# yanivw12/gs2mesh

Hardware: AMD Instinct MI355X
Metric: stereo-pair renders/sec + TSDF Mvoxel-updates/sec (higher is better)
Workload: dtype f32

## Files before the change

### gs2mesh_amd/_lib.py

```python
from __future__ import annotations

import ctypes as C

import numpy as np
import os

_HERE = os.path.dirname(os.path.abspath(__file__))
LIB_PATH = os.path.join(_HERE, "libgs2mesh_amd.so")

vp = C.c_void_p
i32 = C.c_int
i64 = C.c_int64
f32 = C.c_float
f64 = C.c_double


class Camera(C.Structure):
    _fields_ = [("width", C.c_int32), ("height", C.c_int32), ("tanfovx", f32), ("tanfovy", f32),
                ("viewmatrix", f32 * 16), ("projmatrix", f32 * 16), ("campos", f32 * 3)]


class Gaussians(C.Structure):
    _fields_ = [("P", C.c_int32), ("sh_degree", C.c_int32), ("M", C.c_int32), ("raw", C.c_int32),
                ("xyz", vp), ("scales", vp), ("rotations", vp), ("opacities", vp), ("shs", vp), ("shs_rest", vp)]
# ... 41 lines not shown
    "gs2m_raster_status": (i32, [vp, vp, i32, C.POINTER(i64), C.POINTER(i32), C.POINTER(i64)]),
    "gs2m_raster_stage_times": (i32, [vp, vp, C.POINTER(f64), C.POINTER(i64)]),
    "gs2m_raster_blend_cycles": (i32, [vp, vp, C.POINTER(C.c_uint64)]),
    "gs2m_raster_download_geometry": (i32, [vp, vp, i32, i32, vp, vp, vp, vp, vp, vp]),
    "gs2m_raster_download_binning": (i32, [vp, vp, i32, i64, vp, C.c_int32, vp]),
    "gs2m_tsdf_extract_count": (i32, [vp, vp, C.POINTER(i64)]),
    "gs2m_tsdf_extract": (i32, [vp, vp, i64, vp, vp, C.POINTER(i64)]),
    "gs2m_tsdf_extract_indexed": (i32, [vp, vp, i64, vp, vp, vp, C.POINTER(i64)]),
    "gs2m_stereo_depth_occlusion": (i32, [vp, vp, i32, i32, f64, f64, vp, vp, vp]),
    "gs2m_stereo_sgm_scratch_bytes": (i64, [i32, i32, i32]),
    "gs2m_stereo_sgm": (i32, [vp, vp, i32, i32, i32, i32, i32, vp, vp, vp, i64, vp, vp]),
    "gs2m_knn_scratch_bytes": (i64, [i32]),
    "gs2m_knn_mean_dist2": (i32, [i32, vp, vp, vp, i64, vp, vp]),
    "gs2m_mask_preprocess": (i32, [i32, i32, i32, C.POINTER(vp), C.POINTER(vp), i32, i32, i32, i32, C.POINTER(vp), vp, vp]),
    "gs2m_tsdf_create": (i32, [C.POINTER(vp), f64, f64, i32, i32, i32, i64, i32]),
    "gs2m_tsdf_destroy": (i32, [vp]),
    "gs2m_tsdf_reset": (i32, [vp, vp]),
    "gs2m_tsdf_integrate": (i32, [vp, vp, vp, vp, i32, i32, f64, f64, f64, f64, C.POINTER(f64), f64, f64, f64, vp]),
    "gs2m_tsdf_integrate_batch": (i32, [vp, i32, C.POINTER(vp), C.POINTER(vp), C.POINTER(vp), i32, i32, f64, f64, f64, f64,
                                        C.POINTER(f64), f64, f64, f64, vp]),
    "gs2m_tsdf_set_stage_timing": (i32, [vp, i32]),
    "gs2m_tsdf_stage_times": (i32, [vp, vp, C.POINTER(f64), C.POINTER(i64)]),
    "gs2m_tsdf_status": (i32, [vp, vp, C.POINTER(i64), C.POINTER(i64), C.POINTER(i32)]),
    "gs2m_tsdf_download": (i32, [vp, vp, i64, vp, vp, vp, vp]),
    "gs2m_tsdf_block_keys": (i32, [vp, i64, vp, vp]),
    "gs2m_tsdf_flags_device": (i32, [vp, vp, vp]),
    "gs2m_tsdf_pack_sum": (i32, [vp, vp, i64, vp, vp]),
    "gs2m_tsdf_unpack_sum": (i32, [vp, vp, i64, vp, i32, vp]),
    "gs2m_tsdf_pack": (i32, [vp, vp, i64, i32, vp, vp, vp]),
    "gs2m_tsdf_extract_mesh": (i32, [vp, vp, C.POINTER(i64), C.POINTER(i64)]),
    "gs2m_tsdf_mesh_copy": (i32, [vp, vp, vp, vp, vp, vp]),
    "gs2m_mesh_cluster": (i32, [i32, vp, i64, vp, vp, vp, C.POINTER(i64)]),
    "gs2m_mesh_vertex_normals": (i32, [i32, vp, i64, vp, i64, vp, vp, vp]),
    "gs2m_tsdf_replace": (i32, [vp, vp, i64, i32, vp, vp, vp]),
    "gs2m_tsdf_map_bytes": (i64, [C.POINTER(C.c_int32), i32]),
    "gs2m_tsdf_block_map": (i32, [vp, C.POINTER(C.c_int32), C.POINTER(C.c_int32), i32, i32, i64, i64, i32, vp, vp]),
    "gs2m_tsdf_map_keys": (i32, [vp, C.POINTER(C.c_int32), C.POINTER(C.c_int32), i32, vp, vp, i64, C.POINTER(C.c_uint8), vp]),
    "gs2m_tsdf_unpack": (i32, [vp, vp, i64, i32, vp, vp, i32, vp]),
    "gs2m_png_create": (i32, [C.POINTER(vp), i32]),
    "gs2m_png_destroy": (i32, [vp]),
    "gs2m_png_max_bytes": (i64, [i32, i32, i32]),
    "gs2m_png_encode": (i32, [vp, i32, i32, i32, vp, i64, vp, i64, vp, i32, i32, vp]),
}

SYMBOLS = tuple(_PROTOS)

# ... 94 lines not shown
```

### gs2mesh_amd/csrc/tsdf_api.hip

```cpp
#include <math.h>
#include <stdio.h>
#include <string.h>

#include <mutex>
#include <vector>

#include "../../include/gs2mesh_amd.h"
#include "tsdf_common.h"
#include "tsdf_internal.h"
#include "roctx_ranges.h"

#define HIPCHK(expr)                                                                          \
    do {                                                                                      \
        hipError_t e__ = (expr);                                                              \
        if (e__ != hipSuccess) {                                                              \
            gs2m_set_error("%s failed: %s (%s:%d)", #expr, hipGetErrorString(e__), __FILE__, __LINE__); \
            return 1;                                                                         \
        }                                                                                     \
    } while (0)

struct gs2m_tsdf {
    int device = 0;
    double voxel_length = 0, sdf_trunc = 0, unit_length = 0;
    int color_type = 1, resolution = 16, stride = 4;
// ... 6 lines not shown
    unsigned* d_blk_tris = nullptr;
    unsigned long long* d_ntri = nullptr;
    double* mesh_v = nullptr;
    double* mesh_c = nullptr;
    int* mesh_e = nullptr;
    int* mesh_tri = nullptr;
    int64_t mesh_nv = 0, mesh_nt = 0;
    size_t mesh_cap_v = 0, mesh_cap_t = 0;
    char* mesh_scratch = nullptr;
    size_t mesh_scratch_cap = 0;
    int timing = 0;
    struct EvPair {
        int stage;
        hipEvent_t a, b;
        int frames;
    };
    std::vector<EvPair> ev_live;
    std::vector<hipEvent_t> ev_free;
    TsdfBatchFrame* d_bframes = nullptr;
    static const int kRing = 8;
    TsdfBatchFrame* h_bframes = nullptr;
    hipEvent_t ring_done[8] = {nullptr, nullptr, nullptr, nullptr, nullptr, nullptr, nullptr, nullptr};
    unsigned ring_next = 0;
};

static hipEvent_t tsdf_ev_get(gs2m_tsdf* t) {
    if (!t->ev_free.empty()) {
        hipEvent_t e = t->ev_free.back();
        t->ev_free.pop_back();
        return e;
    }
    hipEvent_t e;
    if (hipEventCreate(&e) != hipSuccess) return nullptr;
    return e;
}

static bool invert4x4(const double* m, double* inv) {
    double a[16];
    a[0] = m[5] * m[10] * m[15] - m[5] * m[11] * m[14] - m[9] * m[6] * m[15] + m[9] * m[7] * m[14] + m[13] * m[6] * m[11] - m[13] * m[7] * m[10];
    a[4] = -m[4] * m[10] * m[15] + m[4] * m[11] * m[14] + m[8] * m[6] * m[15] - m[8] * m[7] * m[14] - m[12] * m[6] * m[11] + m[12] * m[7] * m[10];
    a[8] = m[4] * m[9] * m[15] - m[4] * m[11] * m[13] - m[8] * m[5] * m[15] + m[8] * m[7] * m[13] + m[12] * m[5] * m[11] - m[12] * m[7] * m[9];
    a[12] = -m[4] * m[9] * m[14] + m[4] * m[10] * m[13] + m[8] * m[5] * m[14] - m[8] * m[6] * m[13] - m[12] * m[5] * m[10] + m[12] * m[6] * m[9];
    a[1] = -m[1] * m[10] * m[15] + m[1] * m[11] * m[14] + m[9] * m[2] * m[15] - m[9] * m[3] * m[14] - m[13] * m[2] * m[11] + m[13] * m[3] * m[10];
    a[5] = m[0] * m[10] * m[15] - m[0] * m[11] * m[14] - m[8] * m[2] * m[15] + m[8] * m[3] * m[14] + m[12] * m[2] * m[11] - m[12] * m[3] * m[10];
    a[9] = -m[0] * m[9] * m[15] + m[0] * m[11] * m[13] + m[8] * m[1] * m[15] - m[8] * m[3] * m[13] - m[12] * m[1] * m[11] + m[12] * m[3] * m[9];
    a[13] = m[0] * m[9] * m[14] - m[0] * m[10] * m[13] - m[8] * m[1] * m[14] + m[8] * m[2] * m[13] + m[12] * m[1] * m[10] - m[12] * m[2] * m[9];
// ... 8 lines not shown
    double det = m[0] * a[0] + m[1] * a[4] + m[2] * a[8] + m[3] * a[12];
    if (det == 0) return false;
    det = 1.0 / det;
    for (int i = 0; i < 16; i++) inv[i] = a[i] * det;
    return true;
}

static int zero_state(gs2m_tsdf* t, hipStream_t st, bool whole_pool, long long keep_first = -1) {
    TsdfVolume& V = t->V;
    if (whole_pool) {
        HIPCHK(hipMemsetAsync(V.tsdf, 0, sizeof(float) * (size_t)V.max_blocks * GS2M_TSDF_VOX, st));
        HIPCHK(hipMemsetAsync(V.weight, 0, sizeof(float) * (size_t)V.max_blocks * GS2M_TSDF_VOX, st));
        if (V.rgb) HIPCHK(hipMemsetAsync(V.rgb, 0, sizeof(unsigned) * 3 * (size_t)V.max_blocks * GS2M_TSDF_VOX, st));
        HIPCHK(hipMemsetAsync(V.halo, 0, (size_t)V.max_blocks, st));
    } else if (keep_first < 0) {
        gs2m_launch_tsdf_clear_used(st, V);
    } else {
        gs2m_launch_tsdf_clear_from(st, V, (unsigned)keep_first);
    }
    HIPCHK(hipMemsetAsync(V.hash_keys, 0xff, sizeof(unsigned long long) * (size_t)V.hash_cap, st));
    HIPCHK(hipMemsetAsync(V.hash_vals, 0xff, sizeof(int) * (size_t)V.hash_cap, st));
    HIPCHK(hipMemsetAsync(V.stamp, 0, sizeof(unsigned) * (size_t)V.hash_cap, st));
    HIPCHK(hipMemsetAsync(V.fmask, 0, sizeof(unsigned long long) * (size_t)V.hash_cap, st));
    HIPCHK(hipMemsetAsync(V.counters, 0, sizeof(unsigned) * 4, st));
    HIPCHK(hipMemsetAsync(V.totals, 0, sizeof(unsigned long long), st));
    return 0;
}

extern "C" int gs2m_tsdf_create(gs2m_tsdf** out, double voxel_length, double sdf_trunc, int color_type,
                                int volume_unit_resolution, int depth_sampling_stride, int64_t max_blocks,
                                int device) {
    if (!out) {
        gs2m_set_error("gs2m_tsdf_create: out is NULL");
        return 1;
    }
    if (volume_unit_resolution != GS2M_TSDF_RES) {
        gs2m_set_error("volume_unit_resolution %d not supported (kernels are specialised for 16, Open3D's default)",
                       volume_unit_resolution);
        return 1;
    }
    if (!(voxel_length > 0) || !(sdf_trunc > 0) || depth_sampling_stride < 1 || max_blocks < 1 ||
        max_blocks > (1ll << 30) || (color_type != GS2M_TSDF_COLOR_NONE && color_type != GS2M_TSDF_COLOR_RGB8)) {
        gs2m_set_error("gs2m_tsdf_create: bad argument");
        return 1;
    }
    HIPCHK(hipSetDevice(device));
    gs2m_tsdf* t = new gs2m_tsdf();
// ... 3 lines not shown
    t->unit_length = voxel_length * volume_unit_resolution;
    t->color_type = color_type;
    t->stride = depth_sampling_stride;
    memset(&t->V, 0, sizeof(t->V));
    TsdfVolume& V = t->V;
    V.max_blocks = (unsigned)max_blocks;
    unsigned cap = 1024;
    while ((uint64_t)cap < 2ull * (uint64_t)max_blocks) cap <<= 1;
    V.hash_cap = cap;
    V.has_color = color_type == GS2M_TSDF_COLOR_RGB8;
    const size_t nvox = (size_t)max_blocks * GS2M_TSDF_VOX;
    bool ok = hipMalloc((void**)&V.tsdf, sizeof(float) * nvox) == hipSuccess &&
              hipMalloc((void**)&V.weight, sizeof(float) * nvox) == hipSuccess &&
              (!V.has_color || hipMalloc((void**)&V.rgb, sizeof(unsigned) * 3 * nvox) == hipSuccess) &&
              hipMalloc((void**)&V.block_keys, sizeof(int) * 3 * (size_t)max_blocks) == hipSuccess &&
              hipMalloc((void**)&V.halo, (size_t)max_blocks) == hipSuccess &&
              hipMalloc((void**)&V.hash_keys, sizeof(unsigned long long) * (size_t)cap) == hipSuccess &&
              hipMalloc((void**)&V.hash_vals, sizeof(int) * (size_t)cap) == hipSuccess &&
              hipMalloc((void**)&V.stamp, sizeof(unsigned) * (size_t)cap) == hipSuccess &&
              hipMalloc((void**)&V.touched, sizeof(unsigned) * (size_t)cap) == hipSuccess &&
              hipMalloc((void**)&V.fmask, sizeof(unsigned long long) * (size_t)cap) == hipSuccess &&
              hipMalloc((void**)&t->d_bframes, sizeof(TsdfBatchFrame) * GS2M_TSDF_MAX_BATCH) == hipSuccess &&
              hipHostMalloc((void**)&t->h_bframes, sizeof(TsdfBatchFrame) * GS2M_TSDF_MAX_BATCH * gs2m_tsdf::kRing) == hipSuccess &&
              hipMalloc((void**)&V.counters, sizeof(unsigned) * 4) == hipSuccess &&
              hipMalloc((void**)&V.totals, sizeof(unsigned long long)) == hipSuccess &&
              hipMalloc((void**)&t->d_mc, gs2m_mc_tables_bytes()) == hipSuccess &&
              hipMalloc((void**)&t->d_blk_tris, sizeof(unsigned) * (size_t)max_blocks) == hipSuccess &&
              hipMalloc((void**)&t->d_ntri, sizeof(unsigned long long)) == hipSuccess &&
              hipHostMalloc((void**)&t->h_counters, sizeof(unsigned) * 4) == hipSuccess &&
              hipHostMalloc((void**)&t->h_totals, sizeof(unsigned long long)) == hipSuccess;
    if (!ok) {
        gs2m_set_error("gs2m_tsdf_create: out of device memory for %lld blocks (%.1f MiB)", (long long)max_blocks,
                       (double)nvox * 20.0 / 1048576.0);
        gs2m_tsdf_destroy(t);
        return 1;
    }
    {
        std::vector<unsigned char> tab(gs2m_mc_tables_bytes());
        if (!gs2m_mc_tables_fill(tab.data()) ||
            hipMemcpy(t->d_mc, tab.data(), tab.size(), hipMemcpyHostToDevice) != hipSuccess) {
            gs2m_set_error("gs2m_tsdf_create: marching-cubes table generation failed");
            gs2m_tsdf_destroy(t);
            return 1;
        }
    }
    if (zero_state(t, (hipStream_t)0, true)) {
        gs2m_tsdf_destroy(t);
        return 1;
    }
    HIPCHK(hipStreamSynchronize((hipStream_t)0));
    *out = t;
    return 0;
}

extern "C" int gs2m_tsdf_destroy(gs2m_tsdf* t) {
    if (!t) return 0;
    TsdfVolume& V = t->V;
    (void)hipFree(V.tsdf);
    (void)hipFree(V.weight);
    (void)hipFree(V.rgb);
    (void)hipFree(V.block_keys);
    (void)hipFree(V.halo);
    (void)hipFree(V.hash_keys);
    (void)hipFree(V.hash_vals);
    (void)hipFree(V.stamp);
    (void)hipFree(V.touched);
    (void)hipFree(V.fmask);
    (void)hipFree(t->d_bframes);
    (void)hipHostFree(t->h_bframes);
    for (auto e : t->ring_done)
        if (e) (void)hipEventDestroy(e);
    (void)hipFree(V.counters);
    (void)hipFree(V.totals);
    (void)hipFree(t->d_mc);
    (void)hipFree(t->d_blk_tris);
    (void)hipFree(t->d_ntri);
    (void)hipFree(t->mesh_scratch);
    (void)hipFree(t->mesh_v);
    (void)hipFree(t->mesh_c);
    (void)hipFree(t->mesh_e);
    (void)hipFree(t->mesh_tri);
    (void)hipHostFree(t->h_counters);
    (void)hipHostFree(t->h_totals);
    for (auto& p : t->ev_live) {
        (void)hipEventDestroy(p.a);
        (void)hipEventDestroy(p.b);
    }
    for (auto e : t->ev_free) (void)hipEventDestroy(e);
    delete t;
    return 0;
}
// ... 128 lines not shown
    for (int f0 = 0; f0 < n_frames; f0 += GS2M_TSDF_MAX_BATCH) {
        const int nf = n_frames - f0 < GS2M_TSDF_MAX_BATCH ? n_frames - f0 : GS2M_TSDF_MAX_BATCH;
        const unsigned slot = t->ring_next++ % gs2m_tsdf::kRing;
        if (t->ring_done[slot]) HIPCHK(hipEventSynchronize(t->ring_done[slot]));
        else HIPCHK(hipEventCreateWithFlags(&t->ring_done[slot], hipEventDisableTiming));
        TsdfBatchFrame* hb = t->h_bframes + (size_t)slot * GS2M_TSDF_MAX_BATCH;
        for (int k = 0; k < nf; ++k) {
            const int i = f0 + k;
            if (!depth[i] || (t->V.has_color && !color[i])) {
                gs2m_set_error("gs2m_tsdf_integrate_batch: frame %d has a NULL image", i);
                return 1;
            }
            const unsigned char* m = mask ? mask[i] : nullptr;
            if (fill_frame(t, hb[k].f, width, height, fx, fy, cx, cy, extrinsics_w2c + 16 * (size_t)i, depth_scale, depth_trunc,
                           min_depth, m != nullptr))
                return 1;
            hb[k].depth = depth[i];
            hb[k].color = color ? color[i] : nullptr;
            hb[k].mask = m;
        }
        HIPCHK(hipMemcpyAsync(t->d_bframes, hb, sizeof(TsdfBatchFrame) * nf, hipMemcpyHostToDevice, st));
        HIPCHK(hipEventRecord(t->ring_done[slot], st));
        HIPCHK(hipMemsetAsync(t->V.counters + 1, 0, sizeof(unsigned), st));
        HIPCHK(hipMemsetAsync(t->V.counters + 3, 0, sizeof(unsigned), st));
        hipEvent_t e0 = nullptr, e1 = nullptr, e2 = nullptr, e3 = nullptr;
        if (t->timing) {
            e0 = tsdf_ev_get(t);
            e1 = tsdf_ev_get(t);
            e2 = tsdf_ev_get(t);
            e3 = tsdf_ev_get(t);
        }
        const bool tm = e0 && e1 && e2 && e3;
        if (tm) (void)hipEventRecord(e0, st);
        {
            Gs2mRange rg("gs2m:tsdf_touch_batch");
            gs2m_launch_tsdf_touch_batch(st, t->V, hb[0].f, nf, t->d_bframes);
        }
        if (tm) {
            (void)hipEventRecord(e1, st);
            (void)hipEventRecord(e2, st);
        }
        {
            Gs2mRange rg("gs2m:tsdf_integrate_batch");
            gs2m_launch_tsdf_integrate_batch(st, t->n_cu, t->V, t->d_bframes);
        }
        if (tm) {
            (void)hipEventRecord(e3, st);
            t->ev_live.push_back({0, e0, e1, nf});
            t->ev_live.push_back({1, e2, e3, nf});
        }
    }
    return 0;
}

extern "C" int gs2m_tsdf_set_stage_timing(gs2m_tsdf* t, int enable) {
    if (!t) {
        gs2m_set_error("null handle");
        return 1;
    }
// ... 16 lines not shown
        t->ev_free.push_back(p.a);
        t->ev_free.push_back(p.b);
    }
    t->ev_live.clear();
    return 0;
}

extern "C" int gs2m_tsdf_status(gs2m_tsdf* t, gs2m_stream stream, int64_t* n_blocks, int64_t* block_updates,
                                int* overflow) {
    if (!t) {
        gs2m_set_error("null handle");
        return 1;
    }
    hipStream_t st = (hipStream_t)stream;
    HIPCHK(hipMemcpyAsync(t->h_counters, t->V.counters, sizeof(unsigned) * 4, hipMemcpyDeviceToHost, st));
    HIPCHK(hipMemcpyAsync(t->h_totals, t->V.totals, sizeof(unsigned long long), hipMemcpyDeviceToHost, st));
    HIPCHK(hipStreamSynchronize(st));
    HIPCHK(hipGetLastError());
    unsigned nb = t->h_counters[0];
    if (nb > t->V.max_blocks) nb = t->V.max_blocks;
    if (n_blocks) *n_blocks = nb;
    if (block_updates) *block_updates = (int64_t)t->h_totals[0];
    if (overflow) *overflow = (int)t->h_counters[2];
    return 0;
}

extern "C" int gs2m_tsdf_flags_device(gs2m_tsdf* t, uint32_t* flags_dev, gs2m_stream stream) {
    if (!t || !flags_dev) {
        gs2m_set_error("gs2m_tsdf_flags_device: NULL argument");
        return 1;
    }
    HIPCHK(hipSetDevice(t->device));
    HIPCHK(hipMemcpyAsync(flags_dev, t->V.counters + 2, sizeof(unsigned), hipMemcpyDeviceToDevice, (hipStream_t)stream));
    return 0;
}

extern "C" int gs2m_tsdf_block_keys(gs2m_tsdf* t, int64_t n, int32_t* keys, gs2m_stream stream) {
    if (!t || (n > 0 && !keys) || n < 0 || n > (int64_t)t->V.max_blocks) {
        gs2m_set_error("gs2m_tsdf_block_keys: bad argument");
        return 1;
    }
    if (n == 0) return 0;
    HIPCHK(hipSetDevice(t->device));
    gs2m_launch_tsdf_owned_keys((hipStream_t)stream, (unsigned)n, t->V, keys);
    return 0;
}
// ... 460 lines not shown
```

### gs2mesh_amd/csrc/tsdf_common.h

```cpp
#pragma once
#include "platform.h"

#define GS2M_TSDF_RES 16
#define GS2M_TSDF_VOX 4096
#define GS2M_TSDF_EMPTY 0xffffffffffffffffull
#define GS2M_TSDF_KEY_BIAS (1 << 20)

struct TsdfVolume {
    float* tsdf;
    float* weight;
    unsigned* rgb;
    int* block_keys;
    unsigned char* halo;
    unsigned long long* hash_keys;
    int* hash_vals;
    unsigned* stamp;
    unsigned* touched;
    unsigned long long* fmask;
    unsigned* counters;
    unsigned long long* totals;
    unsigned hash_cap;
    unsigned max_blocks;
    int has_color;
};

struct TsdfFrame {
    double pose[12];
    double fx, fy, cx, cy;
    double unit_length, sdf_trunc, depth_trunc;
    float E[12];
    float fx_f, fy_f, cx_f, cy_f, fx_inv_f, fy_inv_f;
    float voxel_length_f, half_voxel_length_f, sdf_trunc_f, sdf_trunc_inv_f;
    float Es02, Es12, Es22;
    float safe_w, safe_h;
    float depth_scale_f, min_depth_f;
    float depth_trunc_up_f;
    int W, H, stride, nx, ny;
    unsigned frame_id;
    int use_mask, use_min;
};

struct TsdfBatchFrame {
    TsdfFrame f;
    const float* depth;
    const unsigned char* color;
    const unsigned char* mask;
};
// ... 22 lines not shown
```

### gs2mesh_amd/csrc/tsdf_internal.h

```cpp
#pragma once
#include "tsdf_common.h"

void gs2m_launch_tsdf_touch(hipStream_t st, const TsdfVolume& V, const TsdfFrame& f, const float* depth,
                            const unsigned char* mask);
void gs2m_launch_tsdf_integrate(hipStream_t st, int n_wg, const TsdfVolume& V, const TsdfFrame& f,
                                const float* depth, const unsigned char* color, const unsigned char* mask);
void gs2m_launch_tsdf_touch_batch(hipStream_t st, const TsdfVolume& V, const TsdfFrame& f, int n_frames,
                                  const TsdfBatchFrame* frames);
void gs2m_launch_tsdf_integrate_batch(hipStream_t st, int n_wg, const TsdfVolume& V, const TsdfBatchFrame* frames);
void gs2m_launch_tsdf_clear_used(hipStream_t st, const TsdfVolume& V);
void gs2m_launch_tsdf_pack(hipStream_t st, unsigned n, const TsdfVolume& V, const int* keys, int form, float* buf, long long* ibuf);
void gs2m_launch_tsdf_unpack(hipStream_t st, unsigned n, const TsdfVolume& V, const int* keys, int form, const float* buf,
                             const long long* ibuf, int halo);
void gs2m_launch_tsdf_clear_from(hipStream_t st, const TsdfVolume& V, unsigned first);
void gs2m_launch_tsdf_clear_gap(hipStream_t st, const TsdfVolume& V, unsigned upto);
void gs2m_launch_tsdf_owned_keys(hipStream_t st, unsigned n, const TsdfVolume& V, int* keys);
void gs2m_launch_tsdf_block_map(hipStream_t st, const TsdfVolume& V, const int* lo, const int* dim, unsigned char* cells, unsigned n_cells,
                                unsigned flags, unsigned win_hash, int rank, unsigned frames_local, unsigned frames_base);
void gs2m_launch_tsdf_map_keys(hipStream_t st, const int* lo, const int* dim, unsigned char* cells, unsigned n_cells, int* keys, unsigned max_keys);
struct McDevTables;
size_t gs2m_mc_tables_bytes();
bool gs2m_mc_tables_fill(void* host_buf);
void gs2m_launch_mc_count(hipStream_t st, const TsdfVolume& V, const McDevTables* T, unsigned n_blocks,
                          unsigned* blk_tris, unsigned long long* n_total);
void gs2m_launch_mc_emit(hipStream_t st, const TsdfVolume& V, const McDevTables* T, unsigned n_blocks,
                         const unsigned* blk_off, unsigned long long max_tris, double voxel_length, double unit_length,
                         double* vertices, double* colors, int* edge_index);
void gs2m_launch_scan_u32(hipStream_t st, const unsigned* in, unsigned n, unsigned* out, unsigned* scratch);
void gs2m_launch_mesh_weld_count(hipStream_t st, unsigned n, const int* edge_index, int* mins, unsigned long long* hkeys, unsigned* hfirst,
                                 unsigned cap, unsigned* cell_of, unsigned* flag, unsigned* pos, unsigned* scratch, unsigned* bad);
void gs2m_launch_mesh_weld_emit(hipStream_t st, unsigned n, const unsigned* hfirst, const unsigned* cell_of, const unsigned* pos, const double* verts,
// ... 12 lines not shown
```

### gs2mesh_amd/csrc/tsdf_kernels.h

```cpp
#pragma once
#include "tsdf_common.h"

GS2M_DEVICE float tsdf_fetch_depth(const float* __restrict__ depth, const unsigned char* __restrict__ mask,
                                   const TsdfFrame& f, int u, int v) {
    const size_t p = (size_t)v * f.W + u;
    float d = depth[p];
    if (f.use_mask && mask[p] == 0) d = d * 0.0f;
    if (f.use_min && d < f.min_depth_f) d = 0.0f;
    if (f.depth_scale_f != 1.0f) d /= f.depth_scale_f;
    if (d >= f.depth_trunc_up_f) d = 0.0f;
    return d;
}

GS2M_DEVICE unsigned tsdf_find_or_insert(const TsdfVolume& V, unsigned long long key, int bx, int by, int bz) {
    const unsigned mask = V.hash_cap - 1u;
    unsigned h = tsdf_hash(key) & mask;
    for (unsigned probe = 0; probe < V.hash_cap; ++probe, h = (h + 1u) & mask) {
        unsigned long long k = V.hash_keys[h];
        if (k == key) return h;
        if (k == GS2M_TSDF_EMPTY) {
            const unsigned long long prev = atomicCAS(&V.hash_keys[h], GS2M_TSDF_EMPTY, key);
            if (prev == GS2M_TSDF_EMPTY) {
                const unsigned slot = atomicAdd(&V.counters[0], 1u);
                if (slot < V.max_blocks) {
// ... 275 lines not shown
                        rgbp[k] = pix[k] < last_pix ? gs2m_load_u32_unaligned(c)
                                                    : ((unsigned)c[0] | ((unsigned)c[1] << 8) | ((unsigned)c[2] << 16));
                    }
                }
            }
#pragma unroll
            for (int k = 0; k < 4; ++k) {
                if (upd[k]) {
                    bt[vi[k]] = (t[k] * w[k] + tnew[k]) / (w[k] + 1.0f);
                    if (V.has_color) {
                        bc[vi[k]] = c0[k] + (rgbp[k] & 0xffu);
                        bc[GS2M_TSDF_VOX + vi[k]] = c1[k] + ((rgbp[k] >> 8) & 0xffu);
                        bc[2 * GS2M_TSDF_VOX + vi[k]] = c2[k] + ((rgbp[k] >> 16) & 0xffu);
                    }
                    bw[vi[k]] = w[k] + 1.0f;
                }
            }
        }
    }
    if (blockIdx.x == 0 && tid == 0) V.totals[0] += n_touched;
}

GS2M_KERNEL void __launch_bounds__(256)
k_tsdf_integrate_batch(TsdfVolume V, const TsdfBatchFrame* __restrict__ frames) {
    __shared__ float s_p0[16], s_p1[16];
    const int tid = (int)threadIdx.x;
    const int x = (tid >> 4) & 15, y = tid & 15;
    __shared__ unsigned s_it;
    const unsigned n_touched = V.counters[1] * 4u;
    const TsdfFrame& f0 = frames[0].f;
    for (;;) {
        __syncthreads();
        if (tid == 0) s_it = atomicAdd(&V.counters[3], 1u);
        __syncthreads();
        const unsigned it = s_it;
        if (it >= n_touched) break;
        const int zq = (int)(it & 3u);
        const unsigned h = V.touched[it >> 2];
        const unsigned long long key = V.hash_keys[h];
        const int slot = V.hash_vals[h];
        const unsigned long long fm = V.fmask[h];
        if (slot < 0) continue;
        const int bx = (int)((key >> 42) & 0x1fffffull) - GS2M_TSDF_KEY_BIAS;
        const int by = (int)((key >> 21) & 0x1fffffull) - GS2M_TSDF_KEY_BIAS;
        const int bz = (int)(key & 0x1fffffull) - GS2M_TSDF_KEY_BIAS;
        const double ox = (double)bx * f0.unit_length, oy = (double)by * f0.unit_length, oz = (double)bz * f0.unit_length;
        const float p2 = (float)(f0.half_voxel_length_f + oz);
        if (tid < 16) s_p0[tid] = (float)(f0.half_voxel_length_f + f0.voxel_length_f * tid + ox);
        else if (tid < 32) s_p1[tid - 16] = (float)(f0.half_voxel_length_f + f0.voxel_length_f * (tid - 16) + oy);
        __syncthreads();
        const float p0 = s_p0[x], p1 = s_p1[y];
        float* bt = V.tsdf + (size_t)slot * GS2M_TSDF_VOX;
        float* bw = V.weight + (size_t)slot * GS2M_TSDF_VOX;
        unsigned* bc = V.rgb + (size_t)slot * 3 * GS2M_TSDF_VOX;
        const int vi0 = GS2M_TSDF_VINDEX(x, y, 4 * zq);
        float w[4], t[4];
        unsigned c0[4], c1[4], c2[4];
#pragma unroll
        for (int j = 0; j < 4; ++j) {
            w[j] = bw[vi0 + 16 * j];
            t[j] = bt[vi0 + 16 * j];
            c0[j] = c1[j] = c2[j] = 0u;
            if (V.has_color) {
                c0[j] = bc[vi0 + 16 * j];
                c1[j] = bc[GS2M_TSDF_VOX + vi0 + 16 * j];
                c2[j] = bc[2 * GS2M_TSDF_VOX + vi0 + 16 * j];
            }
        }
        struct Probe {
            int fi;
            int pix[4];
            unsigned uv[4];
            float zc[4], d[4];
        };
        auto probe = [&](const int fi, Probe& P) __attribute__((always_inline)) {
            const TsdfBatchFrame& bf = frames[fi];
            const TsdfFrame& f = bf.f;
            const float* __restrict__ depth = bf.depth;
            const unsigned char* __restrict__ mask = bf.mask;
            P.fi = fi;
            float pc0 = f.E[0] * p0 + f.E[1] * p1 + f.E[2] * p2 + f.E[3] * 1.f;
            float pc1 = f.E[4] * p0 + f.E[5] * p1 + f.E[6] * p2 + f.E[7] * 1.f;
            float pc2 = f.E[8] * p0 + f.E[9] * p1 + f.E[10] * p2 + f.E[11] * 1.f;
            for (int s = 0; s < 4 * zq; ++s) {
                pc0 += f.Es02;
// ... 54 lines not shown
                    const float sdf = (dd - P.zc[j]) * mult;
                    if (sdf > -f.sdf_trunc_f) {
                        upd[j] = true;
                        tnew[j] = fminf(1.0f, sdf * f.sdf_trunc_inv_f);
                        if (V.has_color) {
                            const unsigned char* c = color + 3 * (size_t)P.pix[j];
                            rgbp[j] = P.pix[j] < last_pix ? gs2m_load_u32_unaligned(c)
                                                          : ((unsigned)c[0] | ((unsigned)c[1] << 8) | ((unsigned)c[2] << 16));
                        }
                    }
                }
            }
#pragma unroll
            for (int j = 0; j < 4; ++j) {
                if (upd[j]) {
                    t[j] = (t[j] * w[j] + tnew[j]) / (w[j] + 1.0f);
                    c0[j] += rgbp[j] & 0xffu;
                    c1[j] += (rgbp[j] >> 8) & 0xffu;
                    c2[j] += (rgbp[j] >> 16) & 0xffu;
                    w[j] = w[j] + 1.0f;
                }
            }
        };
        unsigned long long todo = fm;
        Probe A, B;
        if (todo != 0ull) {
            probe(__ffsll(todo) - 1, A);
            todo &= todo - 1ull;
            while (todo != 0ull) {
                probe(__ffsll(todo) - 1, B);
                todo &= todo - 1ull;
                apply(A);
                if (todo == 0ull) {
                    A = B;
                    break;
                }
                probe(__ffsll(todo) - 1, A);
                todo &= todo - 1ull;
                apply(B);
                if (todo == 0ull) break;
            }
            apply(A);
        }
#pragma unroll
        for (int j = 0; j < 4; ++j) {
            bw[vi0 + 16 * j] = w[j];
            bt[vi0 + 16 * j] = t[j];
            if (V.has_color) {
                bc[vi0 + 16 * j] = c0[j];
                bc[GS2M_TSDF_VOX + vi0 + 16 * j] = c1[j];
                bc[2 * GS2M_TSDF_VOX + vi0 + 16 * j] = c2[j];
            }
        }
        if (tid == 0 && zq == 0) atomicAdd(&V.totals[0], (unsigned long long)gs2m_popc64(fm));
    }
}

GS2M_KERNEL void __launch_bounds__(256)
k_tsdf_clear_fmask(TsdfVolume V) {
    const unsigned n = V.counters[1];
    for (unsigned i = blockIdx.x * 256u + threadIdx.x; i < n; i += gridDim.x * 256u) V.fmask[V.touched[i]] = 0ull;
}

GS2M_KERNEL void __launch_bounds__(256)
k_tsdf_clear_used(TsdfVolume V) {
    unsigned n = V.counters[0];
    if (n > V.max_blocks) n = V.max_blocks;
    const float4 z = {0.f, 0.f, 0.f, 0.f};
// ... 231 lines not shown
```

### gs2mesh_amd/csrc/tsdf_kernels.hip

```cpp
#include "tsdf_kernels.h"
#include "tsdf_extract.h"
#include "mesh_kernels.h"
#include "tsdf_internal.h"
#include <math.h>

void gs2m_launch_tsdf_touch(hipStream_t st, const TsdfVolume& V, const TsdfFrame& f, const float* depth,
                            const unsigned char* mask) {
    const int n = f.nx * f.ny;
    GS2M_LAUNCH(k_tsdf_touch, dim3((n + 255) / 256), dim3(256), 0, st, V, f, depth, mask);
    GS2M_LAUNCH(k_tsdf_compact, dim3((V.hash_cap + 1023u) / 1024u), dim3(1024), 0, st, V, f.frame_id);
}
void gs2m_launch_tsdf_integrate(hipStream_t st, int n_wg, const TsdfVolume& V, const TsdfFrame& f,
                                const float* depth, const unsigned char* color, const unsigned char* mask) {
    GS2M_LAUNCH(k_tsdf_integrate, dim3(n_wg), dim3(256), 0, st, V, f, depth, color, mask);
}
void gs2m_launch_tsdf_touch_batch(hipStream_t st, const TsdfVolume& V, const TsdfFrame& f, int n_frames,
                                  const TsdfBatchFrame* frames) {
    const int n = f.nx * f.ny;
    GS2M_LAUNCH(k_tsdf_touch_batch, dim3((n + 255) / 256, n_frames), dim3(256), 0, st, V, frames);
    GS2M_LAUNCH(k_tsdf_compact, dim3((V.hash_cap + 1023u) / 1024u), dim3(1024), 0, st, V, 0u);
}
void gs2m_launch_tsdf_integrate_batch(hipStream_t st, int n_cu, const TsdfVolume& V, const TsdfBatchFrame* frames) {
    GS2M_LAUNCH(k_tsdf_integrate_batch, dim3(n_cu * 6), dim3(256), 0, st, V, frames);
    GS2M_LAUNCH(k_tsdf_clear_fmask, dim3(16), dim3(256), 0, st, V);
}
void gs2m_launch_tsdf_clear_used(hipStream_t st, const TsdfVolume& V) {
    GS2M_LAUNCH(k_tsdf_clear_used, dim3(2048), dim3(256), 0, st, V);
}
void gs2m_launch_tsdf_pack(hipStream_t st, unsigned n, const TsdfVolume& V, const int* keys, int form, float* buf, long long* ibuf) {
    if (form == GS2M_XF_SUM_PACKED) GS2M_LAUNCH(k_tsdf_pack<GS2M_XF_SUM_PACKED>, dim3(n), dim3(256), 0, st, V, keys, buf, ibuf);
    else if (form == GS2M_XF_RAW_F32) GS2M_LAUNCH(k_tsdf_pack<GS2M_XF_RAW_F32>, dim3(n), dim3(256), 0, st, V, keys, buf, ibuf);
    else GS2M_LAUNCH(k_tsdf_pack<GS2M_XF_SUM_F32>, dim3(n), dim3(256), 0, st, V, keys, buf, ibuf);
}
void gs2m_launch_tsdf_unpack(hipStream_t st, unsigned n, const TsdfVolume& V, const int* keys, int form, const float* buf,
                             const long long* ibuf, int halo) {
    if (form == GS2M_XF_SUM_PACKED) GS2M_LAUNCH(k_tsdf_unpack<GS2M_XF_SUM_PACKED>, dim3(n), dim3(256), 0, st, V, keys, buf, ibuf, halo);
    else if (form == GS2M_XF_RAW_F32) GS2M_LAUNCH(k_tsdf_unpack<GS2M_XF_RAW_F32>, dim3(n), dim3(256), 0, st, V, keys, buf, ibuf, halo);
    else GS2M_LAUNCH(k_tsdf_unpack<GS2M_XF_SUM_F32>, dim3(n), dim3(256), 0, st, V, keys, buf, ibuf, halo);
}
void gs2m_launch_tsdf_clear_from(hipStream_t st, const TsdfVolume& V, unsigned first) {
    GS2M_LAUNCH(k_tsdf_clear_from, dim3(1024), dim3(256), 0, st, V, first);
}
void gs2m_launch_tsdf_clear_gap(hipStream_t st, const TsdfVolume& V, unsigned upto) {
// ... 89 lines not shown
```

### gs2mesh_amd/integration.py

```python
from __future__ import annotations

import ctypes as C
import enum

import numpy as np

from . import _lib
from .rasterizer import _is_torch, _ptr, _stream_of

try:
    import torch
except Exception:
    torch = None


class TSDFVolumeColorType(enum.IntEnum):
    NoColor = 0
    RGB8 = 1
    Gray32 = 2


class PinholeCameraIntrinsic:
    def __init__(self, width, height, fx, fy, cx, cy):
        self.width, self.height = int(width), int(height)
# ... 150 lines not shown
        E = np.ascontiguousarray(np.stack([np.asarray(e, np.float64).reshape(4, 4) for e in extrinsics]))
        st = _stream_of(keep[0], stream)
        _lib.check(self._lib.gs2m_tsdf_integrate_batch(
            self._h, n, dp, cp if has_color else None, mp if masks is not None else None, intrinsic.width, intrinsic.height,
            intrinsic.fx, intrinsic.fy, intrinsic.cx, intrinsic.cy, E.ctypes.data_as(C.POINTER(C.c_double)),
            float(images[0].depth_scale), float(images[0].depth_trunc), float(min_depth), st), self._lib)
        self.frames_local += n
        self._keep.append(keep)
        if len(self._keep) > 64:
            self.status(stream)

    def status(self, stream=None, raise_on_overflow=True):
        nb, bu, ov = C.c_int64(0), C.c_int64(0), C.c_int(0)
        _lib.check(self._lib.gs2m_tsdf_status(self._h, stream or C.c_void_p(0), C.byref(nb), C.byref(bu),
                                              C.byref(ov)), self._lib)
        self._keep.clear()
        if ov.value and raise_on_overflow:
            what = [n for b, n in ((1, "block pool exhausted (raise max_blocks)"), (2, "hash table full"),
                                   (4, "block index out of the +-2^20 range"),
                                   (8, "a voxel did not fit the packed exchange form (weight > 1023: use payload='f32')")) if ov.value & b]
            raise RuntimeError("TSDF volume overflow: " + ", ".join(what))
        return int(nb.value), int(bu.value), int(ov.value)

    def set_stage_timing(self, enable=True):
        _lib.check(self._lib.gs2m_tsdf_set_stage_timing(self._h, int(bool(enable))), self._lib)

    def stage_times(self, stream=None):
        ms = (C.c_double * 2)()
        cnt = (C.c_int64 * 2)()
        _lib.check(self._lib.gs2m_tsdf_stage_times(self._h, stream or C.c_void_p(0), ms, cnt), self._lib)
        return {name: (ms[i], cnt[i]) for i, name in enumerate(_lib.TSDF_STAGES)}

    @property
    def num_blocks(self):
        return self.status()[0]

    @property
    def voxel_updates(self):
        return self.status()[1] * 4096

    def download(self):
        n = self.status()[0]
        keys = np.zeros((n, 3), np.int32)
        tsdf = np.zeros((n, 4096), np.float32)
        weight = np.zeros((n, 4096), np.float32)
        rgb = np.zeros((n, 4096, 3), np.uint32)
# ... 107 lines not shown
```

### include/gs2mesh_amd.h

```cpp
#ifndef GS2MESH_AMD_H
#define GS2MESH_AMD_H

#include <stddef.h>
#include <stdint.h>

#ifdef __cplusplus
extern "C" {
#endif

#define GS2M_VERSION 600

typedef void* gs2m_stream;


int gs2m_version(void);
const char* gs2m_last_error(void);


typedef struct gs2m_raster gs2m_raster;

enum {
    GS2M_OPT_EXACT_TILE_CULL = 1,
    GS2M_OPT_BLEND_VARIANT = 2,
    GS2M_OPT_DEBUG_SYNC = 3,
// ... 99 lines not shown

int gs2m_tsdf_create(gs2m_tsdf** out, double voxel_length, double sdf_trunc, int color_type,
                     int volume_unit_resolution, int depth_sampling_stride, int64_t max_blocks,
                     int device);
int gs2m_tsdf_destroy(gs2m_tsdf* t);
int gs2m_tsdf_reset(gs2m_tsdf* t, gs2m_stream stream);

int gs2m_tsdf_integrate(gs2m_tsdf* t, const float* depth, const uint8_t* color,
                        const uint8_t* mask, int width, int height, double fx, double fy,
                        double cx, double cy, const double* extrinsic_w2c, double depth_scale,
                        double depth_trunc, double min_depth, gs2m_stream stream);

int gs2m_tsdf_integrate_batch(gs2m_tsdf* t, int n_frames, const float* const* depth, const uint8_t* const* color,
                              const uint8_t* const* mask, int width, int height, double fx, double fy, double cx,
                              double cy, const double* extrinsics_w2c, double depth_scale, double depth_trunc,
                              double min_depth, gs2m_stream stream);

int gs2m_tsdf_set_stage_timing(gs2m_tsdf* t, int enable);
int gs2m_tsdf_stage_times(gs2m_tsdf* t, gs2m_stream stream, double* total_ms, int64_t* launches);

int gs2m_tsdf_status(gs2m_tsdf* t, gs2m_stream stream, int64_t* n_blocks,
                     int64_t* block_updates, int* overflow);

int gs2m_tsdf_flags_device(gs2m_tsdf* t, uint32_t* flags_dev, gs2m_stream stream);

int gs2m_tsdf_download(gs2m_tsdf* t, gs2m_stream stream, int64_t n, int32_t* keys,
                       float* tsdf, float* weight, uint32_t* rgb_sum);

int gs2m_tsdf_block_keys(gs2m_tsdf* t, int64_t n, int32_t* keys, gs2m_stream stream);

int gs2m_tsdf_pack_sum(gs2m_tsdf* t, const int32_t* keys, int64_t n, float* buf, gs2m_stream stream);
int gs2m_tsdf_unpack_sum(gs2m_tsdf* t, const int32_t* keys, int64_t n, const float* buf, int halo,
                         gs2m_stream stream);

#define GS2M_TSDF_MAP_HEADER_BYTES 32
int64_t gs2m_tsdf_map_bytes(const int32_t* dim, int world);
int gs2m_tsdf_block_map(gs2m_tsdf* t, const int32_t* lo, const int32_t* dim, int rank, int world, int64_t frames_local,
                        int64_t frames_base, int flags, uint8_t* cells, gs2m_stream stream);
int gs2m_tsdf_map_keys(gs2m_tsdf* t, const int32_t* lo, const int32_t* dim, int world, uint8_t* cells, int32_t* keys,
                       int64_t max_keys, uint8_t* header_host, gs2m_stream stream);

enum { GS2M_XFORM_SUM_F32 = 0, GS2M_XFORM_RAW_F32 = 1, GS2M_XFORM_SUM_PACKED = 2 };
int gs2m_tsdf_pack(gs2m_tsdf* t, const int32_t* keys, int64_t n, int form, float* buf_f32, int64_t* buf_i64,
                   gs2m_stream stream);
int gs2m_tsdf_unpack(gs2m_tsdf* t, const int32_t* keys, int64_t n, int form, const float* buf_f32,
                     const int64_t* buf_i64, int halo, gs2m_stream stream);
// ... 47 lines not shown
```

Measured before the change: 4125.

## Cull TSDF integration passes using per-tile max depth bounds

Adds a kernel that reduces each frame's depth map into 8x8 tile maxima. The batched integrate kernel then projects each block sub-slab's corners per frame and skips frames whose projected footprint lies entirely behind the observed depth plus truncation. Blocks with no surviving frames skip their voxel loads and stores. The cost is an extra pass over each depth map, per-lane culling math, and an atomic counter update per pass. A new API reads back the run and skipped counters.

```diff
diff --git a/gs2mesh_amd/_lib.py b/gs2mesh_amd/_lib.py
--- a/gs2mesh_amd/_lib.py
+++ b/gs2mesh_amd/_lib.py
@@ -87,6 +87,7 @@
     "gs2m_tsdf_set_stage_timing": (i32, [vp, i32]),
     "gs2m_tsdf_stage_times": (i32, [vp, vp, C.POINTER(f64), C.POINTER(i64)]),
     "gs2m_tsdf_status": (i32, [vp, vp, C.POINTER(i64), C.POINTER(i64), C.POINTER(i32)]),
+    "gs2m_tsdf_cull_counters": (i32, [vp, vp, C.POINTER(i64), C.POINTER(i64)]),
     "gs2m_tsdf_download": (i32, [vp, vp, i64, vp, vp, vp, vp]),
     "gs2m_tsdf_block_keys": (i32, [vp, i64, vp, vp]),
     "gs2m_tsdf_flags_device": (i32, [vp, vp, vp]),
diff --git a/gs2mesh_amd/csrc/tsdf_api.hip b/gs2mesh_amd/csrc/tsdf_api.hip
--- a/gs2mesh_amd/csrc/tsdf_api.hip
+++ b/gs2mesh_amd/csrc/tsdf_api.hip
@@ -52,6 +52,8 @@
     TsdfBatchFrame* h_bframes = nullptr;
     hipEvent_t ring_done[8] = {nullptr, nullptr, nullptr, nullptr, nullptr, nullptr, nullptr, nullptr};
     unsigned ring_next = 0;
+    float* dmax = nullptr;
+    size_t dmax_cap = 0;
 };
 
 static hipEvent_t tsdf_ev_get(gs2m_tsdf* t) {
@@ -106,7 +108,7 @@
     HIPCHK(hipMemsetAsync(V.hash_vals, 0xff, sizeof(int) * (size_t)V.hash_cap, st));
     HIPCHK(hipMemsetAsync(V.stamp, 0, sizeof(unsigned) * (size_t)V.hash_cap, st));
     HIPCHK(hipMemsetAsync(V.fmask, 0, sizeof(unsigned long long) * (size_t)V.hash_cap, st));
-    HIPCHK(hipMemsetAsync(V.counters, 0, sizeof(unsigned) * 4, st));
+    HIPCHK(hipMemsetAsync(V.counters, 0, sizeof(unsigned) * GS2M_TSDF_COUNTERS, st));
     HIPCHK(hipMemsetAsync(V.totals, 0, sizeof(unsigned long long), st));
     return 0;
 }
@@ -156,12 +158,12 @@
               hipMalloc((void**)&V.fmask, sizeof(unsigned long long) * (size_t)cap) == hipSuccess &&
               hipMalloc((void**)&t->d_bframes, sizeof(TsdfBatchFrame) * GS2M_TSDF_MAX_BATCH) == hipSuccess &&
               hipHostMalloc((void**)&t->h_bframes, sizeof(TsdfBatchFrame) * GS2M_TSDF_MAX_BATCH * gs2m_tsdf::kRing) == hipSuccess &&
-              hipMalloc((void**)&V.counters, sizeof(unsigned) * 4) == hipSuccess &&
+              hipMalloc((void**)&V.counters, sizeof(unsigned) * GS2M_TSDF_COUNTERS) == hipSuccess &&
               hipMalloc((void**)&V.totals, sizeof(unsigned long long)) == hipSuccess &&
               hipMalloc((void**)&t->d_mc, gs2m_mc_tables_bytes()) == hipSuccess &&
               hipMalloc((void**)&t->d_blk_tris, sizeof(unsigned) * (size_t)max_blocks) == hipSuccess &&
               hipMalloc((void**)&t->d_ntri, sizeof(unsigned long long)) == hipSuccess &&
-              hipHostMalloc((void**)&t->h_counters, sizeof(unsigned) * 4) == hipSuccess &&
+              hipHostMalloc((void**)&t->h_counters, sizeof(unsigned) * GS2M_TSDF_COUNTERS) == hipSuccess &&
               hipHostMalloc((void**)&t->h_totals, sizeof(unsigned long long)) == hipSuccess;
     if (!ok) {
         gs2m_set_error("gs2m_tsdf_create: out of device memory for %lld blocks (%.1f MiB)", (long long)max_blocks,
@@ -201,6 +203,7 @@
     (void)hipFree(V.touched);
     (void)hipFree(V.fmask);
     (void)hipFree(t->d_bframes);
+    (void)hipFree(t->dmax);
     (void)hipHostFree(t->h_bframes);
     for (auto e : t->ring_done)
         if (e) (void)hipEventDestroy(e);
@@ -375,7 +378,21 @@
         HIPCHK(hipMemcpyAsync(t->d_bframes, hb, sizeof(TsdfBatchFrame) * nf, hipMemcpyHostToDevice, st));
         HIPCHK(hipEventRecord(t->ring_done[slot], st));
         HIPCHK(hipMemsetAsync(t->V.counters + 1, 0, sizeof(unsigned), st));
-        HIPCHK(hipMemsetAsync(t->V.counters + 3, 0, sizeof(unsigned), st));
+        HIPCHK(hipMemsetAsync(t->V.counters + 3, 0, sizeof(unsigned) * 3, st));
+        {
+            const int tw = (width + GS2M_TSDF_CULL_TILE - 1) / GS2M_TSDF_CULL_TILE, th = (height + GS2M_TSDF_CULL_TILE - 1) / GS2M_TSDF_CULL_TILE;
+            const size_t need = (size_t)tw * th * GS2M_TSDF_MAX_BATCH;
+            if (need > t->dmax_cap) {
+                HIPCHK(hipFree(t->dmax));
+                t->dmax = nullptr;
+                t->dmax_cap = 0;
+                HIPCHK(hipMalloc((void**)&t->dmax, sizeof(float) * need));
+                t->dmax_cap = need;
+            }
+            t->V.dmax = t->dmax;
+            t->V.dmax_tw = tw;
+            t->V.dmax_th = th;
+        }
         hipEvent_t e0 = nullptr, e1 = nullptr, e2 = nullptr, e3 = nullptr;
         if (t->timing) {
             e0 = tsdf_ev_get(t);
@@ -388,6 +405,7 @@
         {
             Gs2mRange rg("gs2m:tsdf_touch_batch");
             gs2m_launch_tsdf_touch_batch(st, t->V, hb[0].f, nf, t->d_bframes);
+            gs2m_launch_tsdf_depth_tiles(st, t->V, hb[0].f, nf, t->d_bframes);
         }
         if (tm) {
             (void)hipEventRecord(e1, st);
@@ -450,6 +468,19 @@
     if (n_blocks) *n_blocks = nb;
     if (block_updates) *block_updates = (int64_t)t->h_totals[0];
     if (overflow) *overflow = (int)t->h_counters[2];
+    return 0;
+}
+
+extern "C" int gs2m_tsdf_cull_counters(gs2m_tsdf* t, gs2m_stream stream, int64_t* passes_run, int64_t* passes_skipped) {
+    if (!t) {
+        gs2m_set_error("null handle");
+        return 1;
+    }
+    hipStream_t st = (hipStream_t)stream;
+    HIPCHK(hipMemcpyAsync(t->h_counters + 4, t->V.counters + 4, sizeof(unsigned) * 2, hipMemcpyDeviceToHost, st));
+    HIPCHK(hipStreamSynchronize(st));
+    if (passes_run) *passes_run = (int64_t)t->h_counters[4];
+    if (passes_skipped) *passes_skipped = (int64_t)t->h_counters[5];
     return 0;
 }
 
diff --git a/gs2mesh_amd/csrc/tsdf_common.h b/gs2mesh_amd/csrc/tsdf_common.h
--- a/gs2mesh_amd/csrc/tsdf_common.h
+++ b/gs2mesh_amd/csrc/tsdf_common.h
@@ -19,10 +19,19 @@
     unsigned long long* fmask;
     unsigned* counters;
     unsigned long long* totals;
+    float* dmax;
+    int dmax_tw, dmax_th;
     unsigned hash_cap;
     unsigned max_blocks;
     int has_color;
 };
+#define GS2M_TSDF_COUNTERS 6
+#ifndef GS2M_TSDF_CULL_TILE
+#define GS2M_TSDF_CULL_TILE 8
+#endif
+#ifndef GS2M_TSDF_CULL_MAX_TILES
+#define GS2M_TSDF_CULL_MAX_TILES 64
+#endif
 
 struct TsdfFrame {
     double pose[12];
diff --git a/gs2mesh_amd/csrc/tsdf_internal.h b/gs2mesh_amd/csrc/tsdf_internal.h
--- a/gs2mesh_amd/csrc/tsdf_internal.h
+++ b/gs2mesh_amd/csrc/tsdf_internal.h
@@ -7,6 +7,7 @@
                                 const float* depth, const unsigned char* color, const unsigned char* mask);
 void gs2m_launch_tsdf_touch_batch(hipStream_t st, const TsdfVolume& V, const TsdfFrame& f, int n_frames,
                                   const TsdfBatchFrame* frames);
+void gs2m_launch_tsdf_depth_tiles(hipStream_t st, const TsdfVolume& V, const TsdfFrame& f, int n_frames, const TsdfBatchFrame* frames);
 void gs2m_launch_tsdf_integrate_batch(hipStream_t st, int n_wg, const TsdfVolume& V, const TsdfBatchFrame* frames);
 void gs2m_launch_tsdf_clear_used(hipStream_t st, const TsdfVolume& V);
 void gs2m_launch_tsdf_pack(hipStream_t st, unsigned n, const TsdfVolume& V, const int* keys, int form, float* buf, long long* ibuf);
diff --git a/gs2mesh_amd/csrc/tsdf_kernels.h b/gs2mesh_amd/csrc/tsdf_kernels.h
--- a/gs2mesh_amd/csrc/tsdf_kernels.h
+++ b/gs2mesh_amd/csrc/tsdf_kernels.h
@@ -321,6 +321,78 @@
 }
 
 GS2M_KERNEL void __launch_bounds__(256)
+k_tsdf_depth_tiles(TsdfVolume V, const TsdfBatchFrame* __restrict__ frames, int nbx) {
+    const TsdfBatchFrame& bf = frames[blockIdx.y];
+    const TsdfFrame& f = bf.f;
+    const int ty = (int)(blockIdx.x / (unsigned)nbx);
+    const int u = (int)(blockIdx.x % (unsigned)nbx) * 256 + (int)threadIdx.x;
+    float m = 0.0f;
+    if (u < f.W) {
+#pragma unroll
+        for (int r = 0; r < GS2M_TSDF_CULL_TILE; ++r) {
+            const int v = ty * GS2M_TSDF_CULL_TILE + r;
+            if (v < f.H) m = fmaxf(m, tsdf_fetch_depth(bf.depth, bf.mask, f, u, v));
+        }
+    }
+#pragma unroll
+    for (int s = 1; s < GS2M_TSDF_CULL_TILE; s <<= 1) m = fmaxf(m, gs2m_shfl_xor(m, s));
+    if (u % GS2M_TSDF_CULL_TILE == 0 && u < f.W)
+        V.dmax[((size_t)blockIdx.y * V.dmax_th + ty) * V.dmax_tw + u / GS2M_TSDF_CULL_TILE] = m;
+}
+
+GS2M_DEVICE bool tsdf_cull_pass(const TsdfVolume& V, const TsdfFrame& f, int fi, float x0, float x1, float y0, float y1, float p2,
+                                int kz) {
+    const float k0 = (float)kz, k1 = (float)(kz + 3);
+    float zmin = INFINITY, umin = INFINITY, umax = -INFINITY, vmin = INFINITY, vmax = -INFINITY, S = 0.0f;
+    bool sane = true;
+#pragma unroll
+    for (int c = 0; c < 4; ++c) {
+        const float p0 = (c & 1) ? x1 : x0, p1 = (c & 2) ? y1 : y0;
+        const float b0 = f.E[0] * p0 + f.E[1] * p1 + f.E[2] * p2 + f.E[3] * 1.f;
+        const float b1 = f.E[4] * p0 + f.E[5] * p1 + f.E[6] * p2 + f.E[7] * 1.f;
+        const float b2 = f.E[8] * p0 + f.E[9] * p1 + f.E[10] * p2 + f.E[11] * 1.f;
+        S = fmaxf(S, fabsf(f.E[0] * p0) + fabsf(f.E[1] * p1) + fabsf(f.E[2] * p2) + fabsf(f.E[3]));
+        S = fmaxf(S, fabsf(f.E[4] * p0) + fabsf(f.E[5] * p1) + fabsf(f.E[6] * p2) + fabsf(f.E[7]));
+        S = fmaxf(S, fabsf(f.E[8] * p0) + fabsf(f.E[9] * p1) + fabsf(f.E[10] * p2) + fabsf(f.E[11]));
+#pragma unroll
+        for (int e = 0; e < 2; ++e) {
+            const float k = e ? k1 : k0;
+            const float c0 = b0 + k * f.Es02, c1 = b1 + k * f.Es12, c2 = b2 + k * f.Es22;
+            const float uf = c0 * f.fx_f / c2 + f.cx_f + 0.5f;
+            const float vf = c1 * f.fy_f / c2 + f.cy_f + 0.5f;
+            sane = sane && c2 > 0.0f && fabsf(uf) < 1e8f && fabsf(vf) < 1e8f;
+            zmin = fminf(zmin, c2);
+            umin = fminf(umin, uf);
+            umax = fmaxf(umax, uf);
+            vmin = fminf(vmin, vf);
+            vmax = fmaxf(vmax, vf);
+        }
+    }
+    S += 16.0f * fmaxf(fmaxf(fabsf(f.Es02), fabsf(f.Es12)), fabsf(f.Es22));
+    const float delta = S * (1.0f / 262144.0f);
+    const float Q = (float)(f.W > f.H ? f.W : f.H) + fmaxf(fabsf(f.cx_f), fabsf(f.cy_f)) + 2.0f;
+    const float zfloor = 8.0f * delta * fmaxf(fmaxf(fabsf(f.fx_f), fabsf(f.fy_f)), Q);
+    if (!(sane && zmin >= zfloor && zfloor > 0.0f)) return false;
+    int ulo = (int)floorf(fmaxf(umin, -4.0f)) - 1, uhi = (int)floorf(fminf(umax, 70000.0f)) + 1;
+    int vlo = (int)floorf(fmaxf(vmin, -4.0f)) - 1, vhi = (int)floorf(fminf(vmax, 70000.0f)) + 1;
+    ulo = ulo < 0 ? 0 : ulo;
+    vlo = vlo < 0 ? 0 : vlo;
+    uhi = uhi > f.W - 1 ? f.W - 1 : uhi;
+    vhi = vhi > f.H - 1 ? f.H - 1 : vhi;
+    if (uhi < ulo || vhi < vlo) return true;
+    const int tx0 = ulo / GS2M_TSDF_CULL_TILE, tx1 = uhi / GS2M_TSDF_CULL_TILE;
+    const int ty0 = vlo / GS2M_TSDF_CULL_TILE, ty1 = vhi / GS2M_TSDF_CULL_TILE;
+    if ((tx1 - tx0 + 1) * (ty1 - ty0 + 1) > GS2M_TSDF_CULL_MAX_TILES) return false;
+    float d = 0.0f;
+    for (int ty = ty0; ty <= ty1; ++ty) {
+        const float* row = V.dmax + ((size_t)fi * V.dmax_th + ty) * V.dmax_tw;
+        for (int tx = tx0; tx <= tx1; ++tx) d = fmaxf(d, row[tx]);
+    }
+    if (d == 0.0f) return true;
+    return zmin - d >= f.sdf_trunc_f + delta;
+}
+
+GS2M_KERNEL void __launch_bounds__(256)
 k_tsdf_integrate_batch(TsdfVolume V, const TsdfBatchFrame* __restrict__ frames) {
     __shared__ float s_p0[16], s_p1[16];
     const int tid = (int)threadIdx.x;
@@ -349,6 +421,16 @@
         else if (tid < 32) s_p1[tid - 16] = (float)(f0.half_voxel_length_f + f0.voxel_length_f * (tid - 16) + oy);
         __syncthreads();
         const float p0 = s_p0[x], p1 = s_p1[y];
+        unsigned long long rm;
+        {
+            const int lane = tid & 63, wx = (tid >> 6) * 4;
+            bool skip = false;
+            if ((fm >> lane) & 1ull) skip = tsdf_cull_pass(V, frames[lane].f, lane, s_p0[wx], s_p0[wx + 3], s_p1[0], s_p1[15], p2, 4 * zq);
+            rm = fm & ~gs2m_ballot(skip ? 1 : 0);
+            if (lane == 0)
+                atomicAdd(reinterpret_cast<unsigned long long*>(V.counters + 4),
+                          (unsigned long long)gs2m_popc64(rm) | ((unsigned long long)(gs2m_popc64(fm) - gs2m_popc64(rm)) << 32));
+        }
         float* bt = V.tsdf + (size_t)slot * GS2M_TSDF_VOX;
         float* bw = V.weight + (size_t)slot * GS2M_TSDF_VOX;
         unsigned* bc = V.rgb + (size_t)slot * 3 * GS2M_TSDF_VOX;
@@ -357,9 +439,11 @@
         unsigned c0[4], c1[4], c2[4];
 #pragma unroll
         for (int j = 0; j < 4; ++j) {
+            w[j] = t[j] = 0.0f;
+            c0[j] = c1[j] = c2[j] = 0u;
+            if (rm == 0ull) continue;
             w[j] = bw[vi0 + 16 * j];
             t[j] = bt[vi0 + 16 * j];
-            c0[j] = c1[j] = c2[j] = 0u;
             if (V.has_color) {
                 c0[j] = bc[vi0 + 16 * j];
                 c1[j] = bc[GS2M_TSDF_VOX + vi0 + 16 * j];
@@ -460,7 +544,7 @@
                 }
             }
         };
-        unsigned long long todo = fm;
+        unsigned long long todo = rm;
         Probe A, B;
         if (todo != 0ull) {
             probe(__ffsll(todo) - 1, A);
@@ -482,6 +566,7 @@
         }
 #pragma unroll
         for (int j = 0; j < 4; ++j) {
+            if (rm == 0ull) continue;
             bw[vi0 + 16 * j] = w[j];
             bt[vi0 + 16 * j] = t[j];
             if (V.has_color) {
diff --git a/gs2mesh_amd/csrc/tsdf_kernels.hip b/gs2mesh_amd/csrc/tsdf_kernels.hip
--- a/gs2mesh_amd/csrc/tsdf_kernels.hip
+++ b/gs2mesh_amd/csrc/tsdf_kernels.hip
@@ -19,6 +19,10 @@
     const int n = f.nx * f.ny;
     GS2M_LAUNCH(k_tsdf_touch_batch, dim3((n + 255) / 256, n_frames), dim3(256), 0, st, V, frames);
     GS2M_LAUNCH(k_tsdf_compact, dim3((V.hash_cap + 1023u) / 1024u), dim3(1024), 0, st, V, 0u);
+}
+void gs2m_launch_tsdf_depth_tiles(hipStream_t st, const TsdfVolume& V, const TsdfFrame& f, int n_frames, const TsdfBatchFrame* frames) {
+    const int nbx = (f.W + 255) / 256;
+    GS2M_LAUNCH(k_tsdf_depth_tiles, dim3(nbx * V.dmax_th, n_frames), dim3(256), 0, st, V, frames, nbx);
 }
 void gs2m_launch_tsdf_integrate_batch(hipStream_t st, int n_cu, const TsdfVolume& V, const TsdfBatchFrame* frames) {
     GS2M_LAUNCH(k_tsdf_integrate_batch, dim3(n_cu * 6), dim3(256), 0, st, V, frames);
diff --git a/gs2mesh_amd/integration.py b/gs2mesh_amd/integration.py
--- a/gs2mesh_amd/integration.py
+++ b/gs2mesh_amd/integration.py
@@ -196,6 +196,11 @@
             raise RuntimeError("TSDF volume overflow: " + ", ".join(what))
         return int(nb.value), int(bu.value), int(ov.value)
 
+    def cull_counters(self, stream=None):
+        run, skipped = C.c_int64(0), C.c_int64(0)
+        _lib.check(self._lib.gs2m_tsdf_cull_counters(self._h, stream or C.c_void_p(0), C.byref(run), C.byref(skipped)), self._lib)
+        return int(run.value), int(skipped.value)
+
     def set_stage_timing(self, enable=True):
         _lib.check(self._lib.gs2m_tsdf_set_stage_timing(self._h, int(bool(enable))), self._lib)
 
diff --git a/include/gs2mesh_amd.h b/include/gs2mesh_amd.h
--- a/include/gs2mesh_amd.h
+++ b/include/gs2mesh_amd.h
@@ -145,6 +145,8 @@
 int gs2m_tsdf_status(gs2m_tsdf* t, gs2m_stream stream, int64_t* n_blocks,
                      int64_t* block_updates, int* overflow);
 
+int gs2m_tsdf_cull_counters(gs2m_tsdf* t, gs2m_stream stream, int64_t* passes_run, int64_t* passes_skipped);
+
 int gs2m_tsdf_flags_device(gs2m_tsdf* t, uint32_t* flags_dev, gs2m_stream stream);
 
 int gs2m_tsdf_download(gs2m_tsdf* t, gs2m_stream stream, int64_t n, int32_t* keys,
```

Result: no change. 4103 (-0.6%).
